# JianCao92/speaker-diarization

Hardware: AMD Instinct MI355X
Metric: diarized audio throughput (CD gw/BIC + CL hi/BIC) (higher is better)
Workload: dtype f64

## Files before the change

include/spkd.h:

```cpp
#ifndef SPKD_H
#define SPKD_H

#include <stddef.h>
#include <stdint.h>

#ifdef __cplusplus
extern "C" {
#endif

#define SPKD_ABI_VERSION 2
#define SPKD_DIM 39
#define SPKD_REC 820

typedef enum {
    SPKD_OK = 0,
    SPKD_EINVAL = 1,
    SPKD_EHIP = 2,
    SPKD_ENONFINITE = 3,
    SPKD_EOVERFLOW = 4,
    SPKD_ENOMEM = 5
} spkd_status;

typedef enum { SPKD_BIC = 0, SPKD_GLR = 1, SPKD_KL2 = 2, SPKD_KL2_PINV = 3 } spkd_kind;

// ... 160 lines not shown
                             int kind, double lambdac, double threshold, int flags,
                             int32_t *h_merged, double *h_dist, int64_t *h_n_done,
                             int64_t *h_win_cnt, double *h_win_max, double *h_win_min,
                             int64_t *h_det_cnt, double *h_det_max, double *h_det_min);

enum { SPKD_AHC_AUTO = 0, SPKD_AHC_MONO = 1, SPKD_AHC_WIDE = 2 };

typedef struct {
    int32_t variant;
    int32_t kind;
    int32_t max_spk;
    int32_t path;
    double lambdac;
    double threshold;
} spkd_ahc_params;

spkd_status spkd_ahc(spkd_ctx *ctx, const double *d_stats, const int64_t *h_seg_off,
                     int64_t n_problems, const spkd_ahc_params *params,
                     int32_t *h_n_merges, int32_t *h_merge_a, int32_t *h_merge_b,
                     double *h_merge_d, double *h_stat_max, double *h_stat_min);

int64_t spkd_ahc_head_rule(const int64_t *h_seg_off, int64_t n_problems);
spkd_status spkd_last_ahc_head(spkd_ctx *ctx, int64_t *k);

spkd_status spkd_ahc_matrix(spkd_ctx *ctx, const double *d_stats, int64_t n, const spkd_ahc_params *params,
                            const double *d_matrix, double stat_max_in, double stat_min_in,
                            int32_t *h_n_merges, int32_t *h_merge_a, int32_t *h_merge_b,
                            double *h_merge_d, double *h_stat_max, double *h_stat_min);

spkd_status spkd_ahc_fused(spkd_ctx *ctx, const float *d_frames, int64_t n_frames,
                           const double *d_records, int64_t n_records, int64_t *d_line_index,
                           const int64_t *h_seg_off, int64_t n_problems,
                           const int64_t *h_redo_line, const int64_t *h_redo_begin,
                           const int64_t *h_redo_end, int64_t n_redo,
                           const spkd_ahc_params *params,
                           const int32_t **h_n_merges, const int32_t **h_merge_a,
                           const int32_t **h_merge_b, const double **h_merge_d,
                           const int32_t **h_labels);

typedef struct {
    int32_t sample_rate, frame_rate, window_width, n_fft, n_mel, n_cep;
    int32_t cms_left, cms_right;
    int32_t delta_width[2];
    float pre_emph;
    float delta_norm[2];
} spkd_mfcc_params;
// ... 150 lines not shown
```

speaker-diarization_amd/csrc/spkd_cluster.hpp:

```cpp
#pragma once
#include "spkd_device.hpp"
#include "spkd_quad.hpp"
#include "spkd_tri.hpp"
#include "../../include/spkd.h"

namespace spkd {

constexpr double MAXINT_F = 9223372036854775808.0;
constexpr double PEN_UNIT = 39.0 + 0.5 * 39.0 * 40.0;
constexpr int AUX = 3 * DA;
constexpr int ERR_DEGENERATE_MERGE = 2;

__device__ __forceinline__ unsigned long long dkey(double v) {
    unsigned long long b = (unsigned long long)__double_as_longlong(v);
    return (b >> 63) ? ~b : (b | 0x8000000000000000ull);
}
__device__ __forceinline__ double dkey_inv(unsigned long long k) {
    unsigned long long b = (k >> 63) ? (k & 0x7fffffffffffffffull) : ~k;
    return __longlong_as_double((long long)b);
}
template <bool MAXOP>
__device__ __forceinline__ unsigned wave_red_u32(unsigned x) {
    auto op = [](unsigned a, unsigned b) { return MAXOP ? (a > b ? a : b) : (a < b ? a : b); };
    x = op(x, (unsigned)__builtin_amdgcn_update_dpp((int)x, (int)x, 0xB1, 0xf, 0xf, false));
    x = op(x, (unsigned)__builtin_amdgcn_update_dpp((int)x, (int)x, 0x4E, 0xf, 0xf, false));
    x = op(x, (unsigned)__builtin_amdgcn_update_dpp((int)x, (int)x, 0x141, 0xf, 0xf, false));
    x = op(x, (unsigned)__builtin_amdgcn_update_dpp((int)x, (int)x, 0x140, 0xf, 0xf, false));
    const unsigned a = (unsigned)__builtin_amdgcn_readlane((int)x, 0), b = (unsigned)__builtin_amdgcn_readlane((int)x, 16);
    const unsigned c = (unsigned)__builtin_amdgcn_readlane((int)x, 32), d = (unsigned)__builtin_amdgcn_readlane((int)x, 48);
    return op(op(a, b), op(c, d));
}
__device__ __forceinline__ int wave_scan_i32(int x) {
    x += __builtin_amdgcn_update_dpp(0, x, 0x111, 0xf, 0xf, false);
    x += __builtin_amdgcn_update_dpp(0, x, 0x112, 0xf, 0xf, false);
    x += __builtin_amdgcn_update_dpp(0, x, 0x114, 0xf, 0xf, false);
    x += __builtin_amdgcn_update_dpp(0, x, 0x118, 0xf, 0xf, false);
    x += __builtin_amdgcn_update_dpp(0, x, 0x142, 0xa, 0xf, false);
    x += __builtin_amdgcn_update_dpp(0, x, 0x143, 0xc, 0xf, false);
    return x;
}
template <bool MAXOP>
__device__ __forceinline__ unsigned long long wave_red_u64(unsigned long long k) {
    const unsigned hi = (unsigned)(k >> 32), lo = (unsigned)k;
    const unsigned h = wave_red_u32<MAXOP>(hi);
    const unsigned l = wave_red_u32<MAXOP>(hi == h ? lo : (MAXOP ? 0u : 0xffffffffu));
    return ((unsigned long long)h << 32) | l;
}
__device__ __forceinline__ void wave_argmin_key(unsigned long long key, unsigned idx,
                                                unsigned long long& okey, unsigned& oidx) {
    okey = wave_red_u64<false>(key);
// ... 608 lines not shown
        const int fa = al[rc], fd = dirty[rc];
        const unsigned long long mk = __ballot(rl < N && fa && fd);
        if (lane == 0) masks[ch] = mk;
    }
    __syncthreads();
    int ord = 0;
    for (long long ch = 0; ch < n_chunks; ++ch) {
        const long long r0 = ch * WAVE;
        unsigned long long todo = masks[ch];
        while (todo) {
            const int b = __builtin_ctzll(todo);
            todo &= todo - 1;
            if ((ord++ & (AHC_WAVES - 1)) != wave) continue;
            const long long r = r0 + b;
            const RowMin e = scan_row(Dm + r * N, N, [&](long long c) { return al[c] != 0; }, -1, 0.0, lane);
            if (lane == 0) { rmin[r] = e.mv; rarg[r] = e.mc; rnan[r] = e.nc; dirty[r] = 0; }
#ifdef SPKD_PROFILE
            if (lane == 0) atomicAdd(&g_ahc_prof[0], 1ull);
#endif
        }
    }
}

template <bool TWO>
__global__ __launch_bounds__(AHC_TPB) void k_ahc(
        double* __restrict__ ex, double* __restrict__ pk, const int64_t* __restrict__ seg_off,
        int variant, int kind, int max_spk, double lambdac, double threshold,
        double* __restrict__ ld, double* __restrict__ aux,
        double* __restrict__ mat, const int64_t* __restrict__ mat_off,
        int32_t* __restrict__ alive, double* __restrict__ tmp,
        double* __restrict__ rmin_all, int32_t* __restrict__ rcache_all,
        int32_t* __restrict__ out_n, int32_t* __restrict__ out_a, int32_t* __restrict__ out_b,
        double* __restrict__ out_d, unsigned long long* stat_max, unsigned long long* stat_min,
        double* __restrict__ final_max, double* __restrict__ final_min, int* err,
        double* pinv_ws, const int32_t* __restrict__ prob_of_block) {
    extern __shared__ int32_t ids[];
    __shared__ double ldsA[QREC];
    __shared__ unsigned long long red3[AHC_WAVES][3];
    __shared__ unsigned long long s_masks[AHC_MAX_N / WAVE];
    __shared__ int s_cnt[2];
    __shared__ int s_nids;
    __shared__ int s_next;
    __shared__ double s_tmax[AHC_WAVES];
    const int tid = threadIdx.x, lane = lane_id(), wave = tid >> 6;
    const QuadLane L = quad_lane();
    const int p = prob_of_block ? prob_of_block[blockIdx.x] : (int)blockIdx.x;
#ifdef SPKD_PROFILE
    if (tid == 0 && p < AHC_SPAN_PROBS) g_ahc_span[2 * p] = wall_clock64();
#endif
    const int64_t off = seg_off[p];
    const long long N = seg_off[p + 1] - off;
    double* Dm = mat + mat_off[p];
    int32_t* al = alive + off;
    double* ldp = ld + off;
    double* tp = tmp + off;
    double* rmin = rmin_all + off;
    int32_t* rarg = rcache_all + 3 * off;
    int32_t* rnan = rarg + N;
    int32_t* dirty = rnan + N;
    for (long long c = tid; c < N; c += AHC_TPB) { al[c] = 1; dirty[c] = 1; }
    __syncthreads();
    long long m = N;
    int n_merges = 0;
    const long long INF_IDX = 0x7fffffffffffffffLL;
    double fmin = 0.0;
#ifdef SPKD_PROFILE
    unsigned long long ahc_acc[5] = {0ull, 0ull, 0ull, 0ull, 0ull}, ahc_t = clock64();
#define AHC_TICK(i) do { const unsigned long long now_ = clock64(); ahc_acc[i] += now_ - ahc_t; ahc_t = now_; } while (0)
#else
#define AHC_TICK(i) ((void)0)
#endif
    while (true) {
        refresh_rows(Dm, N, al, dirty, rmin, rarg, rnan, s_masks, tid, wave, lane);
        __syncthreads();
        AHC_TICK(0);
        unsigned long long kb = ~0ull, ib = ~0ull, inan = ~0ull;
        for (long long r = tid; r < N; r += AHC_TPB) {
            if (!al[r]) continue;
            const double v = rmin[r];
            const int c = rarg[r], nc = rnan[r];
            if (nc != NO_COL) { const unsigned long long l = (unsigned long long)(r * N + nc); inan = l < inan ? l : inan; }
            if (c != NO_COL) {
                const unsigned long long kv = dkey(v);
                if (kv < kb) { kb = kv; ib = (unsigned long long)(r * N + c); }
            }
        }
        {
            const unsigned long long wk = wave_red_u64<false>(kb);
            const unsigned long long wi = wave_red_u64<false>(kb == wk ? ib : ~0ull);
            const unsigned long long wn = __any(inan != ~0ull) ? wave_red_u64<false>(inan) : ~0ull;
            if (lane == 0) { red3[wave][0] = wk; red3[wave][1] = wi; red3[wave][2] = wn; }
        }
        __syncthreads();
        unsigned long long bk = red3[0][0], bi = red3[0][1], bn = red3[0][2];
#pragma unroll
        for (int w = 1; w < AHC_WAVES; ++w) {
            const unsigned long long ok = red3[w][0], oi = red3[w][1], on = red3[w][2];
            const bool t = ok < bk || (ok == bk && oi < bi);
            bk = t ? ok : bk; bi = t ? oi : bi;
            bn = on < bn ? on : bn;
        }
        const bool has_nan = bn != ~0ull;
        const double mind = has_nan ? __builtin_nan("") : (bi != ~0ull ? dkey_inv(bk) : __builtin_huge_val());
        const long long index = has_nan ? (long long)bn : (bi != ~0ull ? (long long)bi : INF_IDX);
        fmin = mind;
        const bool go = (mind <= threshold) || (max_spk > 0 && m > max_spk);
        if (!go) break;
        AHC_TICK(1);
        const long long r0 = index / N, c0 = index - r0 * N;
        if (r0 == c0) {
            if (tid == 0) atomicOr(err, ERR_DEGENERATE_MERGE);
            break;
        }
        const long long sa = r0 < c0 ? r0 : c0, sb = r0 < c0 ? c0 : r0;
        if (tid < 2) s_cnt[tid] = 0;
        if (tid == 0) { s_nids = 1; s_next = 0; }
        __syncthreads();
        {
            int ca = 0, cb = 0;
            for (long long c = tid; c < sb; c += AHC_TPB) {
                if (al[c]) { cb++; if (c < sa) ca++; }
            }
            ca = __builtin_amdgcn_readlane(wave_scan_i32(ca), WAVE - 1);
            cb = __builtin_amdgcn_readlane(wave_scan_i32(cb), WAVE - 1);
            if (lane == 0 && ca) atomicAdd(&s_cnt[0], ca);
            if (lane == 0 && cb) atomicAdd(&s_cnt[1], cb);
        }
        __syncthreads();
        if (tid == 0) {
            const int64_t o = off + n_merges;
            out_a[o] = s_cnt[0]; out_b[o] = s_cnt[1]; out_d[o] = mind;
            al[sb] = 0;
            ids[0] = (int32_t)sa;
        }
        n_merges++;
        m--;
#ifdef SPKD_PROFILE
        if (tid == 0) atomicAdd(&g_ahc_prof[1], 1ull);
#endif
// ... 42 lines not shown
        const double nA = ldsA[QREC_COUNT_AT];
        if (kind == SPKD_KL2) {
            if (wave == 0) kl2_aux_from_qr(ldsA, aux + (off + sa) * AUX, pinv_ws);
        } else {
            for (;;) {
                int q4 = 0;
                if (lane == 0) q4 = atomicAdd(&s_next, 1);
                const int base = 4 * __builtin_amdgcn_readfirstlane(q4);
                if (base >= nids) break;
                int k = base + L.m;
                const bool valid = k < nids;
                k = valid ? k : nids - 1;
                const int32_t slot = ids[k];
                const double v = quad_pair_det<TWO>(kind, ldsA, nA, A, ex + (off + slot) * QREC, pk + (off + slot) * REC, k == 0, L, err);
                if (valid && L.t == 0) {
                    if (k == 0) ldp[sa] = log(v); else tp[slot] = v;
                }
            }
        }
        __syncthreads();
        AHC_TICK(3);
        double wmax = __builtin_nan(""), wmin = __builtin_nan("");
        const double ldA = ldp[sa];
        for (long long c = tid; c < N; c += AHC_TPB) {
            if (c == sa || !al[c]) continue;
            double d;
            if (kind == SPKD_KL2) {
                d = kl2_from_aux_serial(aux + (off + sa) * AUX, aux + (off + c) * AUX);
            } else {
                const double nC = qr_count(ex + (off + c) * QREC);
                d = finish_distance(kind, lambdac, nA, ldA, nC, ldp[c], log(tp[c]));
            }
            Dm[sa * N + c] = d;
            const double rm0 = rmin[c];
            const int ra0 = rarg[c], rn0 = rnan[c];
            double rm = rm0;
            int ra = ra0, rn = rn0;
            if (variant == 1) Dm[c * N + sa] = d;
            if (row_cache_after_merge(variant, d, (int)sa, (int)sb, rm, ra, rn)) dirty[c] = 1;
            else {
                if (rm != rm0 || ra != ra0) { rmin[c] = rm; rarg[c] = ra; }
                if (rn != rn0) rnan[c] = rn;
            }
            if (variant == 1 && stat_valid(d)) {
                wmax = (wmax != wmax || d > wmax) ? d : wmax;
                wmin = (wmin != wmin || d < wmin) ? d : wmin;
            }
        }
        if (tid == 0) dirty[sa] = 1;
        if (variant == 1) {
            const unsigned long long kmax = wave_red_u64<true>(wmax == wmax ? dkey(wmax) : 0ull);
            const unsigned long long kmin = wave_red_u64<false>(wmin == wmin ? dkey(wmin) : ~0ull);
            if (lane == 0) {
                if (kmax != 0ull) atomicMax(stat_max + p, kmax);
                if (kmin != ~0ull) atomicMin(stat_min + p, kmin);
            }
        }
        __syncthreads();
        AHC_TICK(4);
    }
#ifdef SPKD_PROFILE
    if (tid == 0) for (int i = 0; i < 5; ++i) atomicAdd(&g_ahc_prof[2 + i], ahc_acc[i]);
#endif
    const double mx = final_matrix_max(Dm, N, [&](long long c) { return al[c] != 0; }, s_tmax, tid);
    if (tid == 0) {
        out_n[p] = n_merges;
        final_max[p] = mx;
        final_min[p] = fmin;
#ifdef SPKD_PROFILE
        if (p < AHC_SPAN_PROBS) g_ahc_span[2 * p + 1] = wall_clock64();
#endif
    }
}

constexpr int STEP_WAVES = 4;
constexpr int STEP_WIDE_FROM = 1024;
constexpr int STEP_PARTNERS = 4 * STEP_WAVES - 1;
constexpr int ALIVE_ROUND = 0x7fffffff;
constexpr int STEP_MAX_N = 16384;
constexpr int STEP_IDX_SHIFT = 14;

struct StepState {
    int32_t done, n_merges;
    long long psa;
    double fmin;
    double diag;
};

__host__ __device__ inline unsigned long long step_slot_word(int round, int new_slot, int old_slot) {
// ... 596 lines not shown
```

speaker-diarization_amd/csrc/spkd_hip.hip:

```cpp
#include <hip/hip_runtime.h>

#include <algorithm>
#include <cmath>
#include <cstddef>
#include <cstdio>
#include <cstdlib>
#include <cstring>
#include <functional>
#include <string>
#include <atomic>
#include <thread>
#include <vector>

#include "../../include/spkd.h"
#include "spkd_cd.hpp"
#include "spkd_cluster.hpp"
#include "spkd_device.hpp"
#include "spkd_handoff.hpp"
#include "spkd_merge.hpp"
#include "spkd_stats.hpp"
#include "spkd_post_stats.hpp"
#include "spkd_mfcc.hpp"
#include "spkd_mfcc_batch.hpp"
#include "spkd_resample.hpp"
// ... 9 lines not shown

using namespace spkd;

namespace {
constexpr int N_SLOTS = 72;
enum { PIN_GW_TURNS = 0, PIN_GW_LINES, PIN_AHC_OUT, PIN_VAD_FILES, PIN_VAD_TOKENS, PIN_SUM_IDX, PIN_GAUSS_IDX,
       PIN_GT_TAB, PIN_GT_OUT, PIN_GT_IDX, PIN_UBM_TAB, PIN_UBM_OUT, PIN_CLR_IN, PIN_CLR_OUT, PIN_MD_SEQS, PIN_MD_TOKENS,
       PIN_FB_TAB, PIN_ID_IN, PIN_ID_OUT, PIN_ACC_TAB, PIN_POST_TAB, N_PIN };
}

struct spkd_ctx {
    int device = 0;
    hipStream_t stream = nullptr;
    bool own_stream = false;
    bool gw_lds_ok = false;
    int rs_lds_cap = 0;
    int gw_waves = 0;
    unsigned long long init_keys[2] = {0ull, ~0ull};
    int step_waves = 0;
    int step_partners = 0;
    int64_t last_gw_items = 0;
    int ahc_head = -1;
    int64_t last_ahc_head = 0;
    hipStream_t side = nullptr;
    hipEvent_t ev_fork = nullptr, ev_join = nullptr;
    std::string err;
    int* d_err = nullptr;
    unsigned long long* d_counter = nullptr;
    hipEvent_t ev0 = nullptr, ev1 = nullptr;
    float last_ms = 0.f;
    hipEvent_t ka[SPKD_N_TIMERS] = {}, kb[SPKD_N_TIMERS] = {};
    bool kused[SPKD_N_TIMERS] = {};
    float kms[SPKD_N_TIMERS] = {};
    void* slot[N_SLOTS] = {};
    size_t slot_bytes[N_SLOTS] = {};
    void* pinv_ws = nullptr;
    double* pinv_cur = nullptr;
    void* pin[N_PIN] = {};
    size_t pin_bytes[N_PIN] = {};
    std::vector<int64_t> redo_line, redo_begin, redo_end;
    std::vector<Chunk> redo_chunks;
    std::vector<int64_t> redo_setoff;
    std::vector<int32_t> redo_sets;
};

namespace {
// ... 254 lines not shown
    }
    for (int i = 0; i < SPKD_N_TIMERS; ++i)
        if (hipEventCreate(&c->ka[i]) != hipSuccess || hipEventCreate(&c->kb[i]) != hipSuccess) {
            spkd_destroy(c);
            return SPKD_EHIP;
        }
    int lds_max = 0;
    c->gw_lds_ok = hipDeviceGetAttribute(&lds_max, hipDeviceAttributeMaxSharedMemoryPerBlock, device) == hipSuccess &&
                   Gw<4>::LDS_BYTES <= lds_max &&
                   hipFuncSetAttribute((const void*)k_gw<8>, hipFuncAttributeMaxDynamicSharedMemorySize, Gw<8>::LDS_BYTES) == hipSuccess &&
                   hipFuncSetAttribute((const void*)k_gw<4>, hipFuncAttributeMaxDynamicSharedMemorySize, Gw<4>::LDS_BYTES) == hipSuccess &&
                   hipFuncSetAttribute((const void*)k_gw<2>, hipFuncAttributeMaxDynamicSharedMemorySize, Gw<2>::LDS_BYTES) == hipSuccess &&
                   hipFuncSetAttribute((const void*)k_gw<1>, hipFuncAttributeMaxDynamicSharedMemorySize, Gw<1>::LDS_BYTES) == hipSuccess;
    c->rs_lds_cap = 64 * 1024;
    if (lds_max > c->rs_lds_cap) {
        const int want = lds_max < RS_LDS_MAX ? lds_max : RS_LDS_MAX;
        if (hipFuncSetAttribute((const void*)k_resample, hipFuncAttributeMaxDynamicSharedMemorySize, want) == hipSuccess)
            c->rs_lds_cap = want;
    }
    if (const char* e = getenv("SPKD_GW_WAVES")) c->gw_waves = atoi(e);
    if (const char* e = getenv("SPKD_STEP_WAVES")) { const int v = atoi(e); c->step_waves = (v == 4 || v == 8) ? v : 0; }
    if (const char* e = getenv("SPKD_STEP_PARTNERS")) { const int v = atoi(e); c->step_partners = (v == 3 || v == 7 || v == 15) ? v : 0; }
    if (const char* e = getenv("SPKD_AHC_HEAD")) { const int v = atoi(e); c->ahc_head = v >= 0 ? v : -1; }
    *out = c;
    return SPKD_OK;
}

spkd_status spkd_create(int device, void* stream, spkd_ctx** out) {
    return create_ctx(device, stream, stream != nullptr, out);
}

spkd_status spkd_create_on_stream(int device, void* stream, spkd_ctx** out) {
    return create_ctx(device, stream, true, out);
}

void spkd_destroy(spkd_ctx* c) {
    if (!c) return;
    (void)hipSetDevice(c->device);
    if (c->stream) (void)hipStreamSynchronize(c->stream);
    if (c->side) {
        (void)hipStreamSynchronize(c->side);
        (void)hipStreamDestroy(c->side);
    }
    if (c->ev_fork) (void)hipEventDestroy(c->ev_fork);
    if (c->ev_join) (void)hipEventDestroy(c->ev_join);
    for (int i = 0; i < N_SLOTS; ++i)
// ... 232 lines not shown

void to_quadrec(spkd_ctx* c, const double* d_stats, int64_t n, double* ex) {
    hipLaunchKernelGGL(k_to_quadrec, dim3((unsigned)n), dim3(256), 0, c->stream, d_stats, n, ex);
}

void cluster_prep(spkd_ctx* c, const double* ex, int64_t n, int kind, double* ld, double* aux) {
    const int64_t per_block = kind == SPKD_KL2 ? PT_WAVES : 4 * PT_WAVES;
    const unsigned blocks = (unsigned)((n + per_block - 1) / per_block);
    hipLaunchKernelGGL(k_cluster_prep, dim3(blocks), dim3(PT_WAVES * WAVE), 0, c->stream, ex, n, kind, ld, aux, c->d_err,
                       c->pinv_cur);
}

void matrix_launch(spkd_ctx* c, const AhcPrep& B, const int32_t* d_sched, int64_t grid) {
    if (grid <= 0) return;
    auto kmat = B.kind == SPKD_GLR ? k_matrix<true> : k_matrix<false>;
    hipLaunchKernelGGL(kmat, dim3((unsigned)grid), dim3(MX_WAVES * WAVE), 0, c->stream,
                       (const double*)B.ex, (const double*)B.pk, (const int64_t*)B.seg_off, (const int32_t*)B.d_prob,
                       d_sched, B.variant, B.kind, B.lambdac,
                       (const double*)B.ld, (const double*)B.aux, B.mat, (const int64_t*)B.mat_off,
                       B.smax, B.smin, c->d_err);
}

constexpr int AHC_HEAD_ROUND = 32;
constexpr double AHC_MS_PER_N2 = 2.122e-4;
constexpr double MATRIX_MS_PER_N2 = 5.58e-7;
constexpr int AHC_HEAD_MAX = 32;
constexpr int AHC_RULE_CUS = 256;
int64_t ahc_head_rule(const std::vector<int64_t>& n, int cus) {
    const int64_t n_prob = (int64_t)n.size();
    if (n_prob < 16) return 0;
    auto t = [](int64_t N) { return AHC_MS_PER_N2 * (double)N * (double)N; };
    double sum_all = 0.0;
    for (int64_t N : n) sum_all += (double)N * (double)N;
    const double stage0 = MATRIX_MS_PER_N2 * sum_all + t(n[0]);
    double best = stage0, sum_head = 0.0;
    int64_t best_k = 0;
    for (int64_t k = 1; k <= std::min<int64_t>(AHC_HEAD_MAX, n_prob) && k < cus; ++k) {
        sum_head += (double)n[(size_t)k - 1] * (double)n[(size_t)k - 1];
        const double m_head = MATRIX_MS_PER_N2 * sum_head, m_rest = MATRIX_MS_PER_N2 * (sum_all - sum_head);
        const double rest = k < n_prob ? m_rest * cus / (double)(cus - k) + t(n[(size_t)k]) : 0.0;
        const double stage = m_head + std::max(t(n[0]), rest);
        if (k % AHC_HEAD_ROUND == 0 && stage < best) { best = stage; best_k = k; }
    }
    return stage0 - best < 0.01 * stage0 ? 0 : best_k;
}

spkd_status ahc_prepare(spkd_ctx* c, const double* d_stats, const int64_t* h_seg_off, int64_t n_prob,
                        int variant, int kind, double lambdac, AhcPrep& B, const MatrixPlan& plan = MatrixPlan()) {
// ... 296 lines not shown
spkd_status ahc_impl(spkd_ctx* c, const double* d_stats, const int64_t* h_seg_off, int64_t n_prob,
                     const spkd_ahc_params* P, const MatrixPlan& plan, int32_t* h_n_merges, int32_t* h_merge_a,
                     int32_t* h_merge_b, double* h_merge_d, double* h_stat_max, double* h_stat_min) {
    if (!c || !P || n_prob < 0) return SPKD_EINVAL;
    if (n_prob == 0) return SPKD_OK;
    if (!d_stats || !h_seg_off || !h_n_merges || !h_merge_a || !h_merge_b || !h_merge_d ||
        !h_stat_max || !h_stat_min)
        return fail(c, SPKD_EINVAL, "null argument");
    if ((P->variant != 1 && P->variant != 2) || bad_kind(P->kind))
        return fail(c, SPKD_EINVAL, "bad variant / kind");
    for (int64_t p = 0; p < n_prob; ++p)
        if (h_seg_off[p + 1] - h_seg_off[p] < 1) return fail(c, SPKD_EINVAL, "empty clustering problem");
    int64_t n_max = 0;
    for (int64_t p = 0; p < n_prob; ++p) n_max = std::max<int64_t>(n_max, h_seg_off[p + 1] - h_seg_off[p]);
    if (n_max > AHC_MAX_N) return fail(c, SPKD_EINVAL, "clustering problem larger than 65536 records");
    int path = P->path;
    if (path != SPKD_AHC_MONO && path != SPKD_AHC_WIDE) path = n_prob <= 64 ? SPKD_AHC_WIDE : SPKD_AHC_MONO;
    const size_t lds = (size_t)(n_max + 4) * sizeof(int32_t);
    if (path == SPKD_AHC_MONO && lds > 150 * 1024) path = SPKD_AHC_WIDE;
    if (path == SPKD_AHC_WIDE && n_max > STEP_MAX_N)
        return fail(c, SPKD_EINVAL, "clustering problem larger than 16384 records (wide merge loop)");
    AhcPrep B;
    c->last_ahc_head = 0;
    if (path == SPKD_AHC_MONO && !plan.d_init && plan.row_begin < 0 && P->kind != SPKD_KL2_PINV) {
        B.head_k = c->ahc_head >= 0 ? std::min<int64_t>(c->ahc_head, n_prob) : spkd_ahc_head_rule(h_seg_off, n_prob);
        c->last_ahc_head = B.head_k;
    }
    std::vector<unsigned long long> kmax((size_t)n_prob), kmin((size_t)n_prob);
    std::vector<double> fmax((size_t)n_prob), fmin((size_t)n_prob);
    Call call(c);
    TRY(call.opened);
    spkd_ahc_params Pk;
    TRY(kernel_params(c, P, Pk));
    TRY(ahc_prepare(c, d_stats, h_seg_off, n_prob, P->variant, P->kind, P->lambdac, B, plan));
    const int64_t n_total = B.n_total;
    const size_t nt = (size_t)n_total, np = (size_t)n_prob;
    double *d_merge_d, *d_tmp, *d_rmin, *d_fmax, *d_fmin;
    int32_t *d_a, *d_b, *d_alive, *d_rcache, *d_n;
    TRY(carve(c, scratch, S_AHC_OUT, [&](Layout L) {
        return L.part(d_merge_d, nt).part(d_tmp, nt).part(d_rmin, nt).part(d_fmax, np).part(d_fmin, np)
            .part(d_a, nt).part(d_b, nt).part(d_alive, nt).part(d_rcache, 3 * nt).part(d_n, np).bytes();
    }));
    if (path == SPKD_AHC_MONO) {
        auto kahc = P->kind == SPKD_GLR ? k_ahc<true> : k_ahc<false>;
        if (lds > 48 * 1024)
            (void)hipFuncSetAttribute((const void*)kahc, hipFuncAttributeMaxDynamicSharedMemorySize, (int)lds);
        auto merge_loops = [&](hipStream_t on, int64_t grid, const int32_t* blocks, int64_t largest) {
            hipLaunchKernelGGL(kahc, dim3((unsigned)grid), dim3(AHC_TPB), (size_t)(largest + 4) * sizeof(int32_t), on,
                               B.ex, B.pk, (const int64_t*)B.seg_off, P->variant, P->kind, P->max_spk, P->lambdac,
                               P->threshold, B.ld, B.aux, B.mat, (const int64_t*)B.mat_off, d_alive, d_tmp,
                               d_rmin, d_rcache, d_n, d_a, d_b, d_merge_d, B.smax, B.smin, d_fmax, d_fmin, c->d_err,
                               c->pinv_cur, blocks);
        };
        if (B.head_k > 0) {
            TRY(call.fork());
            (void)hipEventRecord(c->ka[SPKD_T_AHC], c->side);
            merge_loops(c->side, B.head_k, B.d_block_head, B.n_max_head);
            matrix_launch(c, B, B.d_sched, B.grid_rows);
            (void)hipEventRecord(c->kb[SPKD_T_MATRIX], c->stream);
            c->kused[SPKD_T_MATRIX] = true;
            if (n_prob > B.head_k) merge_loops(c->stream, n_prob - B.head_k, B.d_block_rest, B.n_max_rest);
            HIPCHK(c, hipGetLastError());
            TRY(call.join());
            (void)hipEventRecord(c->kb[SPKD_T_AHC], c->stream);
            c->kused[SPKD_T_AHC] = true;
        } else {
            Timer t(c, SPKD_T_AHC);
            merge_loops(c->stream, n_prob, nullptr, n_max);
        }
    } else {
        StepArrays Q;
        void *pe = nullptr, *pp = nullptr;
        TRY(carve(c, scratch, S_STEP_MISC, [&](Layout L) {
            return L.part(Q.sel2, 2 * nt).part(Q.cnt, nt).part(Q.sw, nt).part(Q.state2, 2 * np).part(Q.death, nt).bytes();
        }));
// ... 27 lines not shown
        if (step_lds + 20 * 1024 > 48 * 1024)
            for (int v = 0; v < 3; ++v)
                (void)hipFuncSetAttribute((const void*)kvar[v], hipFuncAttributeMaxDynamicSharedMemorySize, (int)step_lds);
        Timer t(c, SPKD_T_AHC);
        const unsigned row_blocks = (unsigned)((n_max + AHC_WAVES - 1) / AHC_WAVES);
        hipLaunchKernelGGL(k_step_init, dim3(row_blocks, (unsigned)n_prob), dim3(AHC_TPB), 0, c->stream,
                           (const int64_t*)B.seg_off, (const double*)B.mat, (const int64_t*)B.mat_off, Q);
        for (int64_t it = 1; it < n_max; ++it) {
            const int64_t partners = n_max - it - 1;
            const int step_sp = sp_of_round(partners);
            StepKernel kstep = kvar[step_sp == 3 ? 0 : (step_sp == 7 ? 1 : 2)];
            const unsigned blocks = (unsigned)std::max<int64_t>(1, (partners + step_sp - 1) / step_sp) + 1;
            hipLaunchKernelGGL(kstep, dim3(blocks, (unsigned)n_prob), dim3(step_waves * WAVE), step_lds, c->stream,
                               (int)it, (const int64_t*)B.seg_off, P->variant, P->kind, P->max_spk, P->lambdac,
                               P->threshold, B.ld, B.aux, B.mat, (const int64_t*)B.mat_off, Q, d_a, d_b, d_merge_d,
                               B.smax, B.smin, c->d_err, c->pinv_cur);
        }
        hipLaunchKernelGGL(k_step_final, dim3((unsigned)n_prob), dim3(AHC_TPB), 0, c->stream,
                           (int)(n_max - 1), (const int64_t*)B.seg_off, (const double*)B.mat, (const int64_t*)B.mat_off,
                           Q, d_n, d_fmax, d_fmin);
    }
    HIPCHK(c, hipGetLastError());
    HIPCHK(c, hipMemcpyAsync(h_n_merges, d_n, (size_t)n_prob * sizeof(int32_t), hipMemcpyDeviceToHost, c->stream));
    HIPCHK(c, hipMemcpyAsync(h_merge_a, d_a, (size_t)n_total * sizeof(int32_t), hipMemcpyDeviceToHost, c->stream));
    HIPCHK(c, hipMemcpyAsync(h_merge_b, d_b, (size_t)n_total * sizeof(int32_t), hipMemcpyDeviceToHost, c->stream));
    HIPCHK(c, hipMemcpyAsync(h_merge_d, d_merge_d, (size_t)n_total * sizeof(double), hipMemcpyDeviceToHost, c->stream));
    HIPCHK(c, hipMemcpyAsync(kmax.data(), B.smax, (size_t)n_prob * sizeof(unsigned long long), hipMemcpyDeviceToHost, c->stream));
    HIPCHK(c, hipMemcpyAsync(kmin.data(), B.smin, (size_t)n_prob * sizeof(unsigned long long), hipMemcpyDeviceToHost, c->stream));
    HIPCHK(c, hipMemcpyAsync(fmax.data(), d_fmax, (size_t)n_prob * sizeof(double), hipMemcpyDeviceToHost, c->stream));
    HIPCHK(c, hipMemcpyAsync(fmin.data(), d_fmin, (size_t)n_prob * sizeof(double), hipMemcpyDeviceToHost, c->stream));
    const spkd_status st = call.finish();
    for (int64_t p = 0; p < n_prob; ++p) {
        if (P->variant == 1) {
            h_stat_max[p] = key_to_double(kmax[(size_t)p], true);
            h_stat_min[p] = key_to_double(kmin[(size_t)p], false);
        } else {
            h_stat_max[p] = fmax[(size_t)p];
            h_stat_min[p] = fmin[(size_t)p];
        }
    }
    return st;
}
}

spkd_status spkd_ahc(spkd_ctx* c, const double* d_stats, const int64_t* h_seg_off, int64_t n_prob,
                     const spkd_ahc_params* P, int32_t* h_n_merges, int32_t* h_merge_a,
                     int32_t* h_merge_b, double* h_merge_d, double* h_stat_max, double* h_stat_min) {
    return ahc_impl(c, d_stats, h_seg_off, n_prob, P, MatrixPlan(), h_n_merges, h_merge_a, h_merge_b, h_merge_d,
                    h_stat_max, h_stat_min);
}

spkd_status spkd_ahc_matrix(spkd_ctx* c, const double* d_stats, int64_t n, const spkd_ahc_params* P,
                            const double* d_matrix, double stat_max_in, double stat_min_in,
                            int32_t* h_n_merges, int32_t* h_merge_a, int32_t* h_merge_b, double* h_merge_d,
                            double* h_stat_max, double* h_stat_min) {
    if (!c || n < 1) return SPKD_EINVAL;
    if (!d_matrix) return fail(c, SPKD_EINVAL, "ahc_matrix: null matrix");
    const int64_t seg_off[2] = {0, n};
    MatrixPlan plan;
    plan.d_init = d_matrix;
    plan.init_max = stat_max_in;
    plan.init_min = stat_min_in;
    return ahc_impl(c, d_stats, seg_off, 1, P, plan, h_n_merges, h_merge_a, h_merge_b, h_merge_d, h_stat_max, h_stat_min);
}

spkd_status spkd_last_ahc_head(spkd_ctx* c, int64_t* k) {
    if (!c || !k) return SPKD_EINVAL;
    *k = c->last_ahc_head;
    return SPKD_OK;
}

int64_t spkd_ahc_head_rule(const int64_t* h_seg_off, int64_t n_prob) {
    if (!h_seg_off || n_prob < 0) return -1;
    std::vector<int64_t> sizes((size_t)n_prob);
    for (int64_t p = 0; p < n_prob; ++p) sizes[(size_t)p] = h_seg_off[p + 1] - h_seg_off[p];
    std::sort(sizes.begin(), sizes.end(), std::greater<int64_t>());
    return ahc_head_rule(sizes, AHC_RULE_CUS);
}

int64_t spkd_gw_event_capacity(int64_t turn_len, double rate) {
    if (turn_len < 0 || !(rate >= 10.0)) return -1;
    return (int64_t)((double)turn_len / (0.2 * rate)) + 8;
}

int64_t spkd_gw_event_capacity_p(int64_t turn_len, const spkd_cd_params* P) {
    if (turn_len < 0 || !P || !(P->rate >= 10.0) || !(P->winstep >= 1.0)) return -1;
    const double step = std::min(0.2 * P->rate, std::min(0.5 * P->rate, P->winstep));
    return (int64_t)((double)turn_len / step) + 8;
}

int64_t spkd_sw_window_count(int64_t turn_len, double winsize, double winstep) {
// ... 2205 lines not shown
```

speaker-diarization_amd/hipabi.py:

```python
import ctypes as C
import os

import numpy as np

HERE = os.path.dirname(os.path.abspath(__file__))
LIB_PATH = os.environ.get('SPKD_HIP_LIBRARY') or os.path.join(HERE, 'csrc', 'libspkd_hip.so')

SPKD_OK, SPKD_EINVAL, SPKD_EHIP, SPKD_ENONFINITE, SPKD_EOVERFLOW, SPKD_ENOMEM = range(6)
KINDS = {'BIC': 0, 'GLR': 1, 'KL2': 2, 'KL2P': 3}
WANT_GLR, WANT_KL2, WANT_KL2_PINV = 1, 2, 4
MERGE_NO_AHEAD = 1
TIMERS = {n: i for i, n in enumerate(['call', 'chunk_stats', 'reduce_sets', 'pair_terms',
                                        'cluster_prep', 'matrix', 'ahc', 'gw', 'sw', 'merge',
                                        'vad_shift', 'vad_viterbi', 'vad_backtrack', 'gauss_models', 'gauss_loglik',
                                        'post_stats', 'resample',
                                        'gmm_train', 'gmm_seq_loglik', 'ubm_stats', 'clr_link',
                                        'mindur_viterbi', 'mindur_backtrack', 'fb_posterior',
                                        'ident_scores', 'ident_assign', 'bw_accumulate',
                                        'mfcc_static', 'mfcc_post'])}
VAD_TILE = 32
MINDUR_TILE = 32
FB_TILE = 32
POST_CHUNK = 1024
GAUSS_TILE = 64
GAUSS_MODEL = 820
GMM_COMP = 80
GMM_MAX_COMP = 8
GMM_TILE = 64
GMM_CHUNK_TILES = 16
BW_COMP = 40
CLR_MAX_N = 4096
GALLERY_MAX_N = 16384
MFCC_POST_TILE = 128
MFCC_POST_HALO = 4
MFCC_POST_LDS = 61440
MFCC_CMS_MAX = 272
RESAMPLE_TILE = 2048
RESAMPLE_MAX_CH = 8
RESAMPLE_MAX_HALF = 256
RESAMPLE_MAX_TERM = 1 << 20
RESAMPLE_MAX_TAPS = 1 << 22
RESAMPLE_MAX_SPAN = 33281
REC = 820
DIM = 39

EXPORTS = ['spkd_abi_version', 'spkd_create', 'spkd_create_on_stream', 'spkd_destroy', 'spkd_last_error', 'spkd_sync',
           'spkd_malloc', 'spkd_free', 'spkd_memcpy_h2d', 'spkd_memcpy_d2h', 'spkd_memcpy_d2d',
           'spkd_last_kernel_ms', 'spkd_last_gw_items', 'spkd_last_ahc_head', 'spkd_ahc_head_rule', 'spkd_set_stats', 'spkd_pair_terms',
           'spkd_distance_matrix', 'spkd_gw_event_capacity', 'spkd_gw_event_capacity_p', 'spkd_gw', 'spkd_gw_ex', 'spkd_gw_fused', 'spkd_gw_batch', 'spkd_ahc_fused', 'spkd_gather_stats', 'spkd_sum_stats', 'spkd_mfcc', 'spkd_mfcc_batch', 'spkd_resample_batch',
           'spkd_sw_window_count', 'spkd_sw', 'spkd_sw_runs', 'spkd_sw_batch', 'spkd_merge_batch', 'spkd_ahc', 'spkd_ahc_matrix', 'spkd_distance_rows', 'spkd_cluster_in', 'spkd_cluster_in_batch', 'spkd_py2_roundtrip',
           'spkd_labels_from_merges', 'spkd_labels_from_merges_batch', 'spkd_count_flags', 'spkd_gw_lines',
           'spkd_gmm_loglik', 'spkd_vad_viterbi', 'spkd_vad_shift_batch', 'spkd_vad_viterbi_batch',
           'spkd_gauss_models', 'spkd_gauss_loglik', 'spkd_gmm_train', 'spkd_gmm_loglik_seq',
           'spkd_ubm_stats', 'spkd_clr_link', 'spkd_mindur_viterbi_batch', 'spkd_fb_posterior_batch',
           'spkd_clr_identify', 'spkd_bw_accumulate', 'spkd_post_stats']


class CdParams(C.Structure):
    _fields_ = [('kind', C.c_int32), ('trace', C.c_int32), ('lambdac', C.c_double),
                ('threshold', C.c_double), ('winsize', C.c_double), ('winstep', C.c_double),
                ('deltaws', C.c_double), ('rate', C.c_double)]


class CandLog(C.Structure):
    _fields_ = [('turn', C.c_int32), ('coarse', C.c_int32), ('seq', C.c_int64),
                ('start', C.c_double), ('i', C.c_double), ('d', C.c_double),
                ('n1', C.c_int64), ('n2', C.c_int64)]


class GwLinesView(C.Structure):
    _fields_ = [('n_lines', C.c_int64), ('n_redo', C.c_int64), ('n_win', C.c_void_p), ('times', C.c_void_p),
# ... 85 lines not shown
        raise ImportError('HIP extension %s is not built: run `python -c "import __graft_entry__ as g; '
                          'g.build()"` (or make -C speaker-diarization_amd/csrc)' % p)
    _one_hip_runtime()
    lib = C.CDLL(p)
    _check_one_runtime()
    vp, i64, i32, dbl = C.c_void_p, C.c_int64, C.c_int32, C.c_double
    P = C.POINTER
    lib.spkd_abi_version.restype = C.c_int
    lib.spkd_create.argtypes = [C.c_int, vp, P(vp)]
    lib.spkd_create_on_stream.argtypes = [C.c_int, vp, P(vp)]
    lib.spkd_destroy.argtypes = [vp]
    lib.spkd_destroy.restype = None
    lib.spkd_last_error.argtypes = [vp]
    lib.spkd_last_error.restype = C.c_char_p
    lib.spkd_sync.argtypes = [vp]
    lib.spkd_malloc.argtypes = [vp, C.c_size_t, P(vp)]
    lib.spkd_free.argtypes = [vp, vp]
    lib.spkd_memcpy_h2d.argtypes = [vp, vp, vp, C.c_size_t]
    lib.spkd_memcpy_d2h.argtypes = [vp, vp, vp, C.c_size_t]
    lib.spkd_memcpy_d2d.argtypes = [vp, vp, vp, C.c_size_t]
    lib.spkd_last_kernel_ms.argtypes = [vp, C.c_int, P(C.c_float)]
    lib.spkd_last_gw_items.argtypes = [vp, P(C.c_int64)]
    lib.spkd_last_ahc_head.argtypes = [vp, P(C.c_int64)]
    lib.spkd_ahc_head_rule.argtypes = [vp, i64]
    lib.spkd_ahc_head_rule.restype = i64
    lib.spkd_set_stats.argtypes = [vp, vp, i64, vp, vp, vp, i64, i64, vp]
    lib.spkd_pair_terms.argtypes = [vp, vp, vp, vp, i64, C.c_int, vp]
    lib.spkd_distance_matrix.argtypes = [vp, C.c_int, dbl, vp, i64, vp]
    lib.spkd_gw_event_capacity.argtypes = [i64, dbl]
    lib.spkd_gw_event_capacity.restype = i64
    lib.spkd_gw_event_capacity_p.argtypes = [i64, P(CdParams)]
    lib.spkd_gw_event_capacity_p.restype = i64
    lib.spkd_gw.argtypes = [vp, vp, i64, vp, vp, i64, P(CdParams), vp, vp, vp, vp, vp, vp, vp, vp,
                            vp, i64, P(i64)]
    lib.spkd_gw_ex.argtypes = [vp, vp, i64, vp, vp, i64, P(CdParams), vp, C.c_int, vp, vp, vp, vp, vp, vp,
                               vp, vp, i64, P(i64)]
    lib.spkd_gw_fused.argtypes = [vp, vp, i64, vp, vp, i64, P(CdParams), vp, C.c_int, vp, vp, vp, vp, vp, vp,
                                  vp, vp, vp, i64, P(i64)]
    lib.spkd_gw_batch.argtypes = [vp, vp, i64, vp, vp, i64, P(CdParams), vp, vp, vp, vp, vp, vp, C.c_int, P(GwLinesView)]
    lib.spkd_ahc_fused.argtypes = [vp, vp, i64, vp, i64, vp, vp, i64, vp, vp, vp, i64, P(AhcParams),
                                   P(vp), P(vp), P(vp), P(vp), P(vp)]
    lib.spkd_gather_stats.argtypes = [vp, vp, i64, vp, vp, i64, i64, vp]
    lib.spkd_sum_stats.argtypes = [vp, vp, i64, vp, vp, i64, vp]
    lib.spkd_mfcc.argtypes = [vp, vp, i64, P(MfccParams), vp, vp, vp, vp, vp, vp, P(i64)]
    lib.spkd_mfcc_batch.argtypes = [vp, vp, i64, vp, P(MfccParams), vp, vp, vp, vp, vp, vp, vp]
    lib.spkd_resample_batch.argtypes = [vp, vp, i64, vp, vp, vp, i32, vp, vp, vp, vp]
# ... 188 lines not shown
        except Exception:
            pass

    def check(self, st, allow=()):
        if st != SPKD_OK and st not in allow:
            raise SpkdError(st, self.lib.spkd_last_error(self.h).decode())
        return st

    def last_ms(self, which='call'):
        ms = C.c_float()
        self.check(self.lib.spkd_last_kernel_ms(self.h, TIMERS[which], C.byref(ms)))
        return ms.value

    def last_gw_items(self):
        n = C.c_int64()
        self.check(self.lib.spkd_last_gw_items(self.h, C.byref(n)))
        return int(n.value)

    def last_ahc_head(self):
        k = C.c_int64()
        self.check(self.lib.spkd_last_ahc_head(self.h, C.byref(k)))
        return int(k.value)

    def dev_alloc(self, nbytes):
        p = C.c_void_p()
        self.check(self.lib.spkd_malloc(self.h, nbytes, C.byref(p)))
        return p.value

    def dev_free(self, ptr):
        if ptr:
            self.check(self.lib.spkd_free(self.h, C.c_void_p(ptr)))

    def dev_scratch(self, name, nbytes):
        cache = self.__dict__.setdefault('_dev_scratch', {})
        ptr, cap = cache.get(name, (None, 0))
        if ptr is None or cap < nbytes:
            if ptr is not None:
                self.dev_free(ptr)
            ptr, cap = self.dev_alloc(nbytes), nbytes
            cache[name] = (ptr, cap)
        return ptr

    def h2d(self, dptr, arr):
        arr = np.ascontiguousarray(arr)
        self.check(self.lib.spkd_memcpy_h2d(self.h, C.c_void_p(dptr), _ptr(arr), arr.nbytes))

# ... 526 lines not shown
```

Baseline: 1568.

## Carry the next merge selection through the AHC row update to skip refresh passes

During the merge-row update pass the kernel now tracks the minimum over untouched row caches and over the merged row itself. It computes the merged row's cache entry directly instead of marking it dirty. When no row needed a full rescan, the next iteration reuses this carried selection and skips the refresh_rows pass, the global scan and the block reduction. The cross-wave reduction now uses DPP row reductions over a packed selection struct, and the AHC cost-model constants used for head sizing are retuned. The trade-off is more per-cell bookkeeping, extra shared memory and a per-problem counter copied back to the host.

```diff
diff --git a/include/spkd.h b/include/spkd.h
--- a/include/spkd.h
+++ b/include/spkd.h
@@ -206,6 +206,8 @@
 
 int64_t spkd_ahc_head_rule(const int64_t *h_seg_off, int64_t n_problems);
 spkd_status spkd_last_ahc_head(spkd_ctx *ctx, int64_t *k);
+
+spkd_status spkd_last_ahc_carried(spkd_ctx *ctx, int64_t *n);
 
 spkd_status spkd_ahc_matrix(spkd_ctx *ctx, const double *d_stats, int64_t n, const spkd_ahc_params *params,
                             const double *d_matrix, double stat_max_in, double stat_min_in,
diff --git a/speaker-diarization_amd/csrc/spkd_cluster.hpp b/speaker-diarization_amd/csrc/spkd_cluster.hpp
--- a/speaker-diarization_amd/csrc/spkd_cluster.hpp
+++ b/speaker-diarization_amd/csrc/spkd_cluster.hpp
@@ -20,12 +20,18 @@
     return __longlong_as_double((long long)b);
 }
 template <bool MAXOP>
-__device__ __forceinline__ unsigned wave_red_u32(unsigned x) {
+__device__ __forceinline__ unsigned row_red_u32(unsigned x) {
     auto op = [](unsigned a, unsigned b) { return MAXOP ? (a > b ? a : b) : (a < b ? a : b); };
     x = op(x, (unsigned)__builtin_amdgcn_update_dpp((int)x, (int)x, 0xB1, 0xf, 0xf, false));
     x = op(x, (unsigned)__builtin_amdgcn_update_dpp((int)x, (int)x, 0x4E, 0xf, 0xf, false));
     x = op(x, (unsigned)__builtin_amdgcn_update_dpp((int)x, (int)x, 0x141, 0xf, 0xf, false));
     x = op(x, (unsigned)__builtin_amdgcn_update_dpp((int)x, (int)x, 0x140, 0xf, 0xf, false));
+    return x;
+}
+template <bool MAXOP>
+__device__ __forceinline__ unsigned wave_red_u32(unsigned x) {
+    auto op = [](unsigned a, unsigned b) { return MAXOP ? (a > b ? a : b) : (a < b ? a : b); };
+    x = row_red_u32<MAXOP>(x);
     const unsigned a = (unsigned)__builtin_amdgcn_readlane((int)x, 0), b = (unsigned)__builtin_amdgcn_readlane((int)x, 16);
     const unsigned c = (unsigned)__builtin_amdgcn_readlane((int)x, 32), d = (unsigned)__builtin_amdgcn_readlane((int)x, 48);
     return op(op(a, b), op(c, d));
@@ -680,6 +686,60 @@
     }
 }
 
+struct alignas(16) Sel {
+    static constexpr unsigned NONE = 0xffffffffu;
+    unsigned long long k;
+    unsigned i, n;
+    __device__ __forceinline__ void clear() { k = ~0ull; i = NONE; n = NONE; }
+    __device__ __forceinline__ void take(unsigned base, double v, int c, int nc) {
+        if (nc != NO_COL) { const unsigned l = base + (unsigned)nc; n = l < n ? l : n; }
+        if (c != NO_COL) {
+            const unsigned long long kv = dkey(v);
+            const unsigned l = base + (unsigned)c;
+            if (kv < k || (kv == k && l < i)) { k = kv; i = l; }
+        }
+    }
+    __device__ __forceinline__ void take_cell(double v, int c) { take(0u, v, v == v ? c : NO_COL, v == v ? NO_COL : c); }
+    __device__ __forceinline__ Sel of_wave() const {
+        Sel w;
+        w.k = wave_red_u64<false>(k);
+        w.i = wave_red_u32<false>(k == w.k ? i : NONE);
+        w.n = __any(n != NONE) ? wave_red_u32<false>(n) : NONE;
+        return w;
+    }
+    __device__ __forceinline__ RowMin entry() const {
+        RowMin e;
+        e.mv = i != NONE ? dkey_inv(k) : __builtin_huge_val();
+        e.mc = i != NONE ? (int)i : NO_COL;
+        e.nc = n != NONE ? (int)n : NO_COL;
+        return e;
+    }
+};
+static_assert(AHC_WAVES <= 16, "a DPP row takes the waves' parts of a selection");
+__device__ __forceinline__ void sel_leave(Sel* t, int wave, int lane, const Sel& w) {
+    if (lane == 0) t[wave] = w;
+}
+template <int NS>
+__device__ __forceinline__ void sel_fold(const Sel (*t)[AHC_WAVES], int lane, Sel (&out)[NS]) {
+    static_assert(NS >= 1 && NS <= 4, "a DPP row per selection");
+    const int w = lane & 15, j = lane >> 4;
+    const bool holds = w < AHC_WAVES && j < NS;
+    Sel s = t[holds ? j : 0][holds ? w : 0];
+    if (!holds) s.clear();
+    const unsigned hi = (unsigned)(s.k >> 32), lo = (unsigned)s.k;
+    const unsigned rh = row_red_u32<false>(hi);
+    const unsigned rl = row_red_u32<false>(hi == rh ? lo : Sel::NONE);
+    const unsigned ri = row_red_u32<false>(hi == rh && lo == rl ? s.i : Sel::NONE);
+    const unsigned rn = row_red_u32<false>(s.n);
+#pragma unroll
+    for (int q = 0; q < NS; ++q) {
+        out[q].k = ((unsigned long long)(unsigned)__builtin_amdgcn_readlane((int)rh, 16 * q) << 32) |
+                   (unsigned)__builtin_amdgcn_readlane((int)rl, 16 * q);
+        out[q].i = (unsigned)__builtin_amdgcn_readlane((int)ri, 16 * q);
+        out[q].n = (unsigned)__builtin_amdgcn_readlane((int)rn, 16 * q);
+    }
+}
+
 template <bool TWO>
 __global__ __launch_bounds__(AHC_TPB) void k_ahc(
         double* __restrict__ ex, double* __restrict__ pk, const int64_t* __restrict__ seg_off,
@@ -691,10 +751,13 @@
         int32_t* __restrict__ out_n, int32_t* __restrict__ out_a, int32_t* __restrict__ out_b,
         double* __restrict__ out_d, unsigned long long* stat_max, unsigned long long* stat_min,
         double* __restrict__ final_max, double* __restrict__ final_min, int* err,
-        double* pinv_ws, const int32_t* __restrict__ prob_of_block) {
+        double* pinv_ws, const int32_t* __restrict__ prob_of_block,
+        int carry, int32_t* __restrict__ out_carried) {
     extern __shared__ int32_t ids[];
     __shared__ double ldsA[QREC];
-    __shared__ unsigned long long red3[AHC_WAVES][3];
+    __shared__ Sel red3[1][AHC_WAVES];
+    __shared__ Sel s_carry[2][AHC_WAVES];
+    __shared__ int s_redo;
     __shared__ unsigned long long s_masks[AHC_MAX_N / WAVE];
     __shared__ int s_cnt[2];
     __shared__ int s_nids;
@@ -728,39 +791,30 @@
 #else
 #define AHC_TICK(i) ((void)0)
 #endif
+    Sel sel;
+    bool carried = false;
+    int n_carried = 0;
     while (true) {
-        refresh_rows(Dm, N, al, dirty, rmin, rarg, rnan, s_masks, tid, wave, lane);
-        __syncthreads();
-        AHC_TICK(0);
-        unsigned long long kb = ~0ull, ib = ~0ull, inan = ~0ull;
-        for (long long r = tid; r < N; r += AHC_TPB) {
-            if (!al[r]) continue;
-            const double v = rmin[r];
-            const int c = rarg[r], nc = rnan[r];
-            if (nc != NO_COL) { const unsigned long long l = (unsigned long long)(r * N + nc); inan = l < inan ? l : inan; }
-            if (c != NO_COL) {
-                const unsigned long long kv = dkey(v);
-                if (kv < kb) { kb = kv; ib = (unsigned long long)(r * N + c); }
-            }
-        }
-        {
-            const unsigned long long wk = wave_red_u64<false>(kb);
-            const unsigned long long wi = wave_red_u64<false>(kb == wk ? ib : ~0ull);
-            const unsigned long long wn = __any(inan != ~0ull) ? wave_red_u64<false>(inan) : ~0ull;
-            if (lane == 0) { red3[wave][0] = wk; red3[wave][1] = wi; red3[wave][2] = wn; }
-        }
-        __syncthreads();
-        unsigned long long bk = red3[0][0], bi = red3[0][1], bn = red3[0][2];
-#pragma unroll
-        for (int w = 1; w < AHC_WAVES; ++w) {
-            const unsigned long long ok = red3[w][0], oi = red3[w][1], on = red3[w][2];
-            const bool t = ok < bk || (ok == bk && oi < bi);
-            bk = t ? ok : bk; bi = t ? oi : bi;
-            bn = on < bn ? on : bn;
-        }
-        const bool has_nan = bn != ~0ull;
-        const double mind = has_nan ? __builtin_nan("") : (bi != ~0ull ? dkey_inv(bk) : __builtin_huge_val());
-        const long long index = has_nan ? (long long)bn : (bi != ~0ull ? (long long)bi : INF_IDX);
+        if (!carried) {
+            refresh_rows(Dm, N, al, dirty, rmin, rarg, rnan, s_masks, tid, wave, lane);
+            __syncthreads();
+            AHC_TICK(0);
+            sel.clear();
+            for (long long r = tid; r < N; r += AHC_TPB) {
+                if (!al[r]) continue;
+                sel.take((unsigned)(r * N), rmin[r], rarg[r], rnan[r]);
+            }
+            sel_leave(red3[0], wave, lane, sel.of_wave());
+            __syncthreads();
+            Sel f[1];
+            sel_fold(red3, lane, f);
+            sel = f[0];
+        } else {
+            n_carried++;
+        }
+        const bool has_nan = sel.n != Sel::NONE;
+        const double mind = has_nan ? __builtin_nan("") : (sel.i != Sel::NONE ? dkey_inv(sel.k) : __builtin_huge_val());
+        const long long index = has_nan ? (long long)sel.n : (sel.i != Sel::NONE ? (long long)sel.i : INF_IDX);
         fmin = mind;
         const bool go = (mind <= threshold) || (max_spk > 0 && m > max_spk);
         if (!go) break;
@@ -772,7 +826,7 @@
         }
         const long long sa = r0 < c0 ? r0 : c0, sb = r0 < c0 ? c0 : r0;
         if (tid < 2) s_cnt[tid] = 0;
-        if (tid == 0) { s_nids = 1; s_next = 0; }
+        if (tid == 0) { s_nids = 1; s_next = 0; s_redo = 0; }
         __syncthreads();
         {
             int ca = 0, cb = 0;
@@ -861,6 +915,11 @@
         AHC_TICK(3);
         double wmax = __builtin_nan(""), wmin = __builtin_nan("");
         const double ldA = ldp[sa];
+        const double diag = Dm[sa * N + sa];
+        Sel row;
+        bool redo = false;
+        row.clear();
+        sel.clear();
         for (long long c = tid; c < N; c += AHC_TPB) {
             if (c == sa || !al[c]) continue;
             double d;
@@ -876,17 +935,18 @@
             double rm = rm0;
             int ra = ra0, rn = rn0;
             if (variant == 1) Dm[c * N + sa] = d;
-            if (row_cache_after_merge(variant, d, (int)sa, (int)sb, rm, ra, rn)) dirty[c] = 1;
+            row.take_cell(d, (int)c);
+            if (row_cache_after_merge(variant, d, (int)sa, (int)sb, rm, ra, rn)) { dirty[c] = 1; redo = true; }
             else {
                 if (rm != rm0 || ra != ra0) { rmin[c] = rm; rarg[c] = ra; }
                 if (rn != rn0) rnan[c] = rn;
+                sel.take((unsigned)(c * N), rm, ra, rn);
             }
             if (variant == 1 && stat_valid(d)) {
                 wmax = (wmax != wmax || d > wmax) ? d : wmax;
                 wmin = (wmin != wmin || d < wmin) ? d : wmin;
             }
         }
-        if (tid == 0) dirty[sa] = 1;
         if (variant == 1) {
             const unsigned long long kmax = wave_red_u64<true>(wmax == wmax ? dkey(wmax) : 0ull);
             const unsigned long long kmin = wave_red_u64<false>(wmin == wmin ? dkey(wmin) : ~0ull);
@@ -895,7 +955,21 @@
                 if (kmin != ~0ull) atomicMin(stat_min + p, kmin);
             }
         }
+        sel_leave(s_carry[0], wave, lane, sel.of_wave());
+        sel_leave(s_carry[1], wave, lane, row.of_wave());
+        if (__any(redo) && lane == 0) s_redo = 1;
         __syncthreads();
+        Sel f[2];
+        sel_fold(s_carry, lane, f);
+        f[1].take_cell(diag, (int)sa);
+        const RowMin e = f[1].entry();
+        if (tid == 0) { rmin[sa] = e.mv; rarg[sa] = e.mc; rnan[sa] = e.nc; }
+        sel = f[0];
+        sel.take((unsigned)(sa * N), e.mv, e.mc, e.nc);
+        carried = carry != 0 && __builtin_amdgcn_readfirstlane(s_redo) == 0;
+#ifdef SPKD_PROFILE
+        if (tid == 0 && carried) atomicAdd(&g_ahc_prof[7], 1ull);
+#endif
         AHC_TICK(4);
     }
 #ifdef SPKD_PROFILE
@@ -904,6 +978,7 @@
     const double mx = final_matrix_max(Dm, N, [&](long long c) { return al[c] != 0; }, s_tmax, tid);
     if (tid == 0) {
         out_n[p] = n_merges;
+        out_carried[p] = n_carried;
         final_max[p] = mx;
         final_min[p] = fmin;
 #ifdef SPKD_PROFILE
diff --git a/speaker-diarization_amd/csrc/spkd_hip.hip b/speaker-diarization_amd/csrc/spkd_hip.hip
--- a/speaker-diarization_amd/csrc/spkd_hip.hip
+++ b/speaker-diarization_amd/csrc/spkd_hip.hip
@@ -55,6 +55,8 @@
     int64_t last_gw_items = 0;
     int ahc_head = -1;
     int64_t last_ahc_head = 0;
+    int ahc_carry = 1;
+    int64_t last_ahc_carried = 0;
     hipStream_t side = nullptr;
     hipEvent_t ev_fork = nullptr, ev_join = nullptr;
     std::string err;
@@ -355,6 +357,7 @@
     if (const char* e = getenv("SPKD_STEP_WAVES")) { const int v = atoi(e); c->step_waves = (v == 4 || v == 8) ? v : 0; }
     if (const char* e = getenv("SPKD_STEP_PARTNERS")) { const int v = atoi(e); c->step_partners = (v == 3 || v == 7 || v == 15) ? v : 0; }
     if (const char* e = getenv("SPKD_AHC_HEAD")) { const int v = atoi(e); c->ahc_head = v >= 0 ? v : -1; }
+    if (const char* e = getenv("SPKD_AHC_CARRY")) c->ahc_carry = atoi(e) != 0;
     *out = c;
     return SPKD_OK;
 }
@@ -633,8 +636,8 @@
 }
 
 constexpr int AHC_HEAD_ROUND = 32;
-constexpr double AHC_MS_PER_N2 = 2.122e-4;
-constexpr double MATRIX_MS_PER_N2 = 5.58e-7;
+constexpr double AHC_MS_PER_N2 = 2.027e-4;
+constexpr double MATRIX_MS_PER_N2 = 5.48e-7;
 constexpr int AHC_HEAD_MAX = 32;
 constexpr int AHC_RULE_CUS = 256;
 int64_t ahc_head_rule(const std::vector<int64_t>& n, int cus) {
@@ -977,6 +980,7 @@
         return fail(c, SPKD_EINVAL, "clustering problem larger than 16384 records (wide merge loop)");
     AhcPrep B;
     c->last_ahc_head = 0;
+    c->last_ahc_carried = 0;
     if (path == SPKD_AHC_MONO && !plan.d_init && plan.row_begin < 0 && P->kind != SPKD_KL2_PINV) {
         B.head_k = c->ahc_head >= 0 ? std::min<int64_t>(c->ahc_head, n_prob) : spkd_ahc_head_rule(h_seg_off, n_prob);
         c->last_ahc_head = B.head_k;
@@ -994,7 +998,7 @@
     int32_t *d_a, *d_b, *d_alive, *d_rcache, *d_n;
     TRY(carve(c, scratch, S_AHC_OUT, [&](Layout L) {
         return L.part(d_merge_d, nt).part(d_tmp, nt).part(d_rmin, nt).part(d_fmax, np).part(d_fmin, np)
-            .part(d_a, nt).part(d_b, nt).part(d_alive, nt).part(d_rcache, 3 * nt).part(d_n, np).bytes();
+            .part(d_a, nt).part(d_b, nt).part(d_alive, nt).part(d_rcache, 3 * nt).part(d_n, 2 * np).bytes();
     }));
     if (path == SPKD_AHC_MONO) {
         auto kahc = P->kind == SPKD_GLR ? k_ahc<true> : k_ahc<false>;
@@ -1005,7 +1009,7 @@
                                B.ex, B.pk, (const int64_t*)B.seg_off, P->variant, P->kind, P->max_spk, P->lambdac,
                                P->threshold, B.ld, B.aux, B.mat, (const int64_t*)B.mat_off, d_alive, d_tmp,
                                d_rmin, d_rcache, d_n, d_a, d_b, d_merge_d, B.smax, B.smin, d_fmax, d_fmin, c->d_err,
-                               c->pinv_cur, blocks);
+                               c->pinv_cur, blocks, c->ahc_carry, d_n + np);
         };
         if (B.head_k > 0) {
             TRY(call.fork());
@@ -1079,6 +1083,9 @@
     }
     HIPCHK(c, hipGetLastError());
     HIPCHK(c, hipMemcpyAsync(h_n_merges, d_n, (size_t)n_prob * sizeof(int32_t), hipMemcpyDeviceToHost, c->stream));
+    std::vector<int32_t> carried(path == SPKD_AHC_MONO ? np : 0);
+    if (!carried.empty())
+        HIPCHK(c, hipMemcpyAsync(carried.data(), d_n + np, np * sizeof(int32_t), hipMemcpyDeviceToHost, c->stream));
     HIPCHK(c, hipMemcpyAsync(h_merge_a, d_a, (size_t)n_total * sizeof(int32_t), hipMemcpyDeviceToHost, c->stream));
     HIPCHK(c, hipMemcpyAsync(h_merge_b, d_b, (size_t)n_total * sizeof(int32_t), hipMemcpyDeviceToHost, c->stream));
     HIPCHK(c, hipMemcpyAsync(h_merge_d, d_merge_d, (size_t)n_total * sizeof(double), hipMemcpyDeviceToHost, c->stream));
@@ -1087,6 +1094,7 @@
     HIPCHK(c, hipMemcpyAsync(fmax.data(), d_fmax, (size_t)n_prob * sizeof(double), hipMemcpyDeviceToHost, c->stream));
     HIPCHK(c, hipMemcpyAsync(fmin.data(), d_fmin, (size_t)n_prob * sizeof(double), hipMemcpyDeviceToHost, c->stream));
     const spkd_status st = call.finish();
+    if (st == SPKD_OK) for (int32_t k : carried) c->last_ahc_carried += k;
     for (int64_t p = 0; p < n_prob; ++p) {
         if (P->variant == 1) {
             h_stat_max[p] = key_to_double(kmax[(size_t)p], true);
@@ -1124,6 +1132,12 @@
 spkd_status spkd_last_ahc_head(spkd_ctx* c, int64_t* k) {
     if (!c || !k) return SPKD_EINVAL;
     *k = c->last_ahc_head;
+    return SPKD_OK;
+}
+
+spkd_status spkd_last_ahc_carried(spkd_ctx* c, int64_t* n) {
+    if (!c || !n) return SPKD_EINVAL;
+    *n = c->last_ahc_carried;
     return SPKD_OK;
 }
 
diff --git a/speaker-diarization_amd/hipabi.py b/speaker-diarization_amd/hipabi.py
--- a/speaker-diarization_amd/hipabi.py
+++ b/speaker-diarization_amd/hipabi.py
@@ -46,7 +46,7 @@
 
 EXPORTS = ['spkd_abi_version', 'spkd_create', 'spkd_create_on_stream', 'spkd_destroy', 'spkd_last_error', 'spkd_sync',
            'spkd_malloc', 'spkd_free', 'spkd_memcpy_h2d', 'spkd_memcpy_d2h', 'spkd_memcpy_d2d',
-           'spkd_last_kernel_ms', 'spkd_last_gw_items', 'spkd_last_ahc_head', 'spkd_ahc_head_rule', 'spkd_set_stats', 'spkd_pair_terms',
+           'spkd_last_kernel_ms', 'spkd_last_gw_items', 'spkd_last_ahc_head', 'spkd_last_ahc_carried', 'spkd_ahc_head_rule', 'spkd_set_stats', 'spkd_pair_terms',
            'spkd_distance_matrix', 'spkd_gw_event_capacity', 'spkd_gw_event_capacity_p', 'spkd_gw', 'spkd_gw_ex', 'spkd_gw_fused', 'spkd_gw_batch', 'spkd_ahc_fused', 'spkd_gather_stats', 'spkd_sum_stats', 'spkd_mfcc', 'spkd_mfcc_batch', 'spkd_resample_batch',
            'spkd_sw_window_count', 'spkd_sw', 'spkd_sw_runs', 'spkd_sw_batch', 'spkd_merge_batch', 'spkd_ahc', 'spkd_ahc_matrix', 'spkd_distance_rows', 'spkd_cluster_in', 'spkd_cluster_in_batch', 'spkd_py2_roundtrip',
            'spkd_labels_from_merges', 'spkd_labels_from_merges_batch', 'spkd_count_flags', 'spkd_gw_lines',
@@ -178,6 +178,7 @@
     lib.spkd_last_kernel_ms.argtypes = [vp, C.c_int, P(C.c_float)]
     lib.spkd_last_gw_items.argtypes = [vp, P(C.c_int64)]
     lib.spkd_last_ahc_head.argtypes = [vp, P(C.c_int64)]
+    lib.spkd_last_ahc_carried.argtypes = [vp, P(C.c_int64)]
     lib.spkd_ahc_head_rule.argtypes = [vp, i64]
     lib.spkd_ahc_head_rule.restype = i64
     lib.spkd_set_stats.argtypes = [vp, vp, i64, vp, vp, vp, i64, i64, vp]
@@ -412,6 +413,11 @@
         self.check(self.lib.spkd_last_ahc_head(self.h, C.byref(k)))
         return int(k.value)
 
+    def last_ahc_carried(self):
+        n = C.c_int64()
+        self.check(self.lib.spkd_last_ahc_carried(self.h, C.byref(n)))
+        return int(n.value)
+
     def dev_alloc(self, nbytes):
         p = C.c_void_p()
         self.check(self.lib.spkd_malloc(self.h, nbytes, C.byref(p)))
```

Result: no change. 1579 (median of 2 runs) (+0.7%).
